# benjaminrwilson/range-view-3d-detection

Hardware: AMD Instinct MI355X
Metric: sweeps/sec (fwd+bwd, 64x2048x5 range image) (higher is better)
Workload: dtype bf16

## Files before the change

include/rv3d.h:

```cpp
#ifndef RV3D_H_
#define RV3D_H_

#include <stdint.h>

#ifdef __cplusplus
extern "C" {
#endif

typedef void* rvStream;

int rv_version(void);
const char* rv_last_error(void);

typedef struct {
    int32_t kh, kw;
    int32_t stride_w;
    int32_t pad_h, pad_w;
    int32_t cu, cv;
} rvTapGeom;

int32_t rv_pad_channels(int32_t c);

int64_t rv_packed_weight_bytes(const rvTapGeom* g);

int rv_pack_weight(const rvTapGeom* g, const float* T, void* gather_w, void* scatter_w, rvStream stream);

int64_t rv_pack_batch_entry_bytes(void);
int rv_pack_batch_fill(const rvTapGeom* g, const float* T, void* gather_w, void* scatter_w, void* host_entries);
int rv_pack_batch(const void* dev_table, int32_t n_entries, rvStream stream);

int rv_fold_geom(const rvTapGeom* g, rvTapGeom* folded);
int rv_pack_weight_folded(const rvTapGeom* g, const float* T, void* gather_w_folded, rvStream stream);
int rv_pack_batch_fill_folded(const rvTapGeom* g, const float* T, void* gather_w_folded, void* host_entry);
int rv_unfold_weight_grad(const rvTapGeom* g, const float* dT_folded, float* dT, int32_t accumulate, rvStream stream);

int rv_unpack_weight_grad(const rvTapGeom* g, const float* packed, float* dT, int32_t accumulate, rvStream stream);

#define RV_IN_AFFINE 1
#define RV_IN_RELU 2
#define RV_OUT_F32 4
#define RV_OUT_BIAS 8
#define RV_OUT_STATS 16
#define RV_OUT_ACCUM 32
#define RV_OUT_RELU 64
#define RV_OUT_RES_RELU 256
#define RV_WGRAD_TORCH_LAYOUT 128
#define RV_SEL_SMALL_GRIDS (1 << 20)
#define RV_SEL_SMALL_GRIDS6 (1 << 21)
#define RV_SEL_NO_GEN6 (1 << 22)
#define RV_SEL_NO_GEN5 (1 << 23)
#define RV_SEL_NO_POINTWISE (1 << 24)
#define RV_SEL_NO_POINTWISE_BWD (1 << 25)
#define RV_SEL_MASK (63 << 20)

typedef struct {
    int32_t N, H, Wu, Wv;
    int32_t ld_src, ld_dst;
    int32_t flags;
} rvTapShape;

int32_t rv_tap_stats_rows(const rvTapGeom* g, const rvTapShape* s, int32_t scatter);
int rv_tap_launch_info(const rvTapGeom* g, const rvTapShape* s, int32_t scatter, int32_t* host_info);
#define RV_STATS_SCRATCH_ROWS 128

int rv_tap_gather(const rvTapGeom* g, const rvTapShape* s, const void* V, const float* in_scale,
                  const float* in_shift, const void* gather_w, const float* bias, void* U,
                  float* stats_partial, rvStream stream);

int rv_tap_scatter(const rvTapGeom* g, const rvTapShape* s, const void* U, const float* in_scale,
                   const float* in_shift, const void* scatter_w, const float* bias, void* V,
                   float* stats_partial, rvStream stream);

int rv_tap_residual(const rvTapGeom* g, const rvTapShape* s, int32_t scatter, const void* src, const void* w, const float* bias,
                    const void* res, int32_t ld_res, void* dst, rvStream stream);

typedef struct rvBnbEpilogue {
    const void* y;
    int32_t ld_y;
    int32_t flags;
    const float* scale;
    const float* shift;
    const float* mean;
    const float* invstd;
    float* partial;
} rvBnbEpilogue;
int32_t rv_tap_bnb_rows(const rvTapGeom* g, const rvTapShape* s, int32_t scatter);
int rv_tap_data_grad_bnb(const rvTapGeom* g, const rvTapShape* s, int32_t scatter, const void* dout, const void* w, void* dx,
                         const rvBnbEpilogue* e, rvStream stream);

int64_t rv_tap_wgrad_workspace_bytes(const rvTapGeom* g, const rvTapShape* s);
int rv_tap_wgrad_info(const rvTapGeom* g, const rvTapShape* s, int32_t* host_info);
int rv_tap_wgrad(const rvTapGeom* g, const rvTapShape* s, const void* U, int32_t ld_u, const void* V, int32_t ld_v,
                 const float* in_scale, const float* in_shift, int32_t v_affine, float* dT_packed,
                 void* workspace, rvStream stream);

int rv_reduce_rows(const float* partial, int32_t rows, int32_t cols, float* out, rvStream stream);
int rv_reduce_rows_count(const float* partial, int32_t rows, int32_t cols, float count, float* out, float* out_copy, rvStream stream);
int rv_bn_finalize(const float* partial, int32_t rows, int32_t c, int64_t count, const float* gamma,
                   const float* beta, float eps, float momentum, float* running_mean, float* running_var,
                   float* scale, float* shift, float* mean, float* invstd, rvStream stream);
int rv_bn_fold_eval(int32_t c, const float* gamma, const float* beta, const float* running_mean,
                    const float* running_var, float eps, float* scale, float* shift, rvStream stream);

#define RV_EW_RELU_A 1
#define RV_EW_RELU_B 2
#define RV_EW_RELU_OUT 4
// ... 354 lines not shown
```

range_view_3d_detection_amd/_lib.py:

```python

from __future__ import annotations

import ctypes
import os
import re
import functools
from typing import Dict, List, Optional, Tuple

import torch

_HERE = os.path.dirname(os.path.abspath(__file__))
LIB_PATH = os.environ.get("RV3D_LIB") or os.path.join(_HERE, "librv3d_hip.so")
LIB_PATH_F16 = os.environ.get("RV3D_LIB_F16") or os.path.join(_HERE, "librv3d_hip_f16.so")
HEADER_PATH = os.path.join(os.path.dirname(_HERE), "include", "rv3d.h")
COMPANION_HEADERS = ("rv3d_render.h",)
OPTIM_HEADERS = ("rv3d_optim.h",)
AVERAGE_ENTRIES = ("rv_adamw_step_groups_avg", "rv_average_tensors")

IN_AFFINE, IN_RELU, OUT_F32, OUT_BIAS, OUT_STATS, OUT_ACCUM, OUT_RELU = 1, 2, 4, 8, 16, 32, 64
OUT_RES_RELU = 256
WGRAD_TORCH_LAYOUT = 128
SEL_SMALL_GRIDS, SEL_SMALL_GRIDS6, SEL_NO_GEN6, SEL_NO_GEN5, SEL_NO_POINTWISE, SEL_NO_POINTWISE_BWD = 1 << 20, 1 << 21, 1 << 22, 1 << 23, 1 << 24, 1 << 25
SELECT = 0
EW_RELU_A, EW_RELU_B, EW_RELU_OUT = 1, 2, 4
BNB_RELU_Z, BNB_RES_ACCUM, BNB_Y_FROM_INPUT = 1, 2, 4
ADAM_AMSGRAD, ADAM_MAXIMIZE = 1, 2
WNMS_MERGE_SUPPRESSED, WNMS_SCORE_KEEPER, WNMS_NMS_GE, WNMS_MERGE_GE = 1, 2, 4, 8
EW_PASS_COMBINE, EW_PASS_MASK_GRAD, EW_PASS_BN_FINALIZE, EW_PASS_BWD_REDUCE, EW_PASS_BWD_REDUCE_PAIR, EW_PASS_BWD_FINALIZE, EW_PASS_BWD_APPLY, EW_PASS_BWD_APPLY_PAIR = range(8)
EW_FORM_COMB, EW_FORM_ROWS, EW_FORM_OCTET, EW_FORM_LEAN, EW_FORM_FUSED_FINALIZE, EW_FORM_TWO_STAGE = range(1, 7)
STATS_SCRATCH_ROWS = 128


class TapGeom(ctypes.Structure):
    _fields_ = [(n, ctypes.c_int32) for n in ("kh", "kw", "stride_w", "pad_h", "pad_w", "cu", "cv")]


class TapShape(ctypes.Structure):
    _fields_ = [(n, ctypes.c_int32) for n in ("N", "H", "Wu", "Wv", "ld_src", "ld_dst", "flags")]

    def __init__(self, *args, **kw) -> None:
        super().__init__(*args, **kw)
        self.flags |= SELECT


class select:

    def __init__(self, flags: int) -> None:
        self.flags = flags

    def __enter__(self):
        global SELECT
        self.old, SELECT = SELECT, SELECT | self.flags
        return self

    def __exit__(self, *exc):
        global SELECT
        SELECT = self.old


class BnbEpilogue(ctypes.Structure):

    _fields_ = [("y", ctypes.c_void_p), ("ld_y", ctypes.c_int32), ("flags", ctypes.c_int32), ("scale", ctypes.c_void_p), ("shift", ctypes.c_void_p),
                ("mean", ctypes.c_void_p), ("invstd", ctypes.c_void_p), ("partial", ctypes.c_void_p)]


class TargetLevel(ctypes.Structure):

    _fields_ = [("stride", ctypes.c_int32), ("use_range", ctypes.c_int32), ("lower", ctypes.c_double), ("upper", ctypes.c_double)]


class TargetOut(ctypes.Structure):

    _fields_ = [(n, ctypes.c_void_p) for n in ("labels", "panoptics", "reg_targets", "points_per_obj")]


# ... 271 lines not shown
```

range_view_3d_detection_amd/csrc/tapconv.h:

```cpp
#pragma once
#include "common.h"

constexpr int kMaxTaps = 24;
constexpr int kMaxPhases = 4;
constexpr int RV_OUT_BNB = 1 << 16;

struct TapTable {
    int32_t ntaps[kMaxPhases];
    int32_t w_first[kMaxPhases];
    int32_t dw_min[kMaxPhases], dw_max[kMaxPhases];
    int32_t w_tile[kMaxPhases];
    int32_t dh_min, rows;
    int8_t dh[kMaxPhases][kMaxTaps];
    int8_t dw[kMaxPhases][kMaxTaps];
    int8_t ky[kMaxPhases][kMaxTaps];
    int8_t kx[kMaxPhases][kMaxTaps];
};

struct TapConvArgs {
    const bf16_t* src;
    void* dst;
    const bf16_t* w;
    const float* in_scale;
    const float* in_shift;
    const float* bias;
    float* stats;
    int32_t N, H, W_src, W_dst;
    int32_t C_src, C_dst;
    int32_t ld_src, ld_dst;
    int32_t phases, step;
    int32_t m_tiles;
    int32_t h_tiles;
    int32_t total_tiles, n_tiles, tiles_per_xcd;
    int32_t lds_a_elems;
    int32_t lds_tab_offset;
    int32_t flags;
    int32_t sel;
    const bf16_t* bnb_y;
    const float *bnb_scale, *bnb_shift, *bnb_mean, *bnb_invstd;
    float* bnb_partial;
    int32_t ld_bnb_y, bnb_flags;
    const bf16_t* res;
    int32_t ld_res;
    int32_t stats_per_wg;
    TapTable tt;
};

int rv_build_tap_table(const rvTapGeom* g, bool scatter, TapTable* tt, int* phases, int* step);

struct TapPlan {
    int gen;
    int bn, ks;
    int mt, nt;
    int epi;
    int pair, slices;
    int grid_x, grid_y;
    size_t lds;
    int stats_rows;
    int bnb_rows;
    int32_t info[4];
    bool scatter;
    TapConvArgs args;
};

bool rv_tapconv2_plan(TapPlan* p);
int rv_tapconv2_launch(const TapPlan& p, hipStream_t stream);
bool rv_tapconv4_plan(TapPlan* p);
int rv_tapconv4_launch(const TapPlan& p, hipStream_t stream);
bool rv_tapconv5_plan(TapPlan* p);
int rv_tapconv5_launch(const TapPlan& p, hipStream_t stream);
bool rv_tapconv6_plan(TapPlan* p);
int rv_tapconv6_launch(const TapPlan& p, hipStream_t stream);
bool rv_pointwise_plan(TapPlan* p);
int rv_pointwise_launch(const TapPlan& p, hipStream_t stream);
```

range_view_3d_detection_amd/csrc/tapconv6.hip:

```cpp
#include <stdlib.h>

#include "common.h"
#include "tapconv.h"

namespace {

constexpr int kTC = 32;
constexpr int kTR = 16;
constexpr int kBK = 32;
constexpr int kBN = 128;
constexpr int kPitch = 36;
constexpr int kHaloRows = 18;
constexpr int kHaloInstr = (kHaloRows * kPitch + 15) / 16;
constexpr int kHaloBytes = kHaloInstr * 1024;
constexpr int kPiece = kBN * kBK * 2;
constexpr int kNRing = 8;
#ifndef RV_T6_AHEAD
#define RV_T6_AHEAD 4
#endif
constexpr int kAhead = RV_T6_AHEAD;
constexpr int kRing = 2 * kHaloBytes;
constexpr int kScratch = kRing + kNRing * kPiece;
constexpr int kTab = kScratch + 1024;
constexpr int kStatAcc = kTab + 32 * 4;
constexpr int kBnbAcc = kStatAcc + 8 * 4 * 16 * 2 * 4;
constexpr int kLds = kBnbAcc + 256 * 4;
constexpr int kMinTaps = kAhead + 2 > 6 ? kAhead + 2 : 6;

__device__ __attribute__((aligned(256))) uint32_t g_zero_page6[64];

typedef __attribute__((address_space(3))) void lds_void_t;
typedef const __attribute__((address_space(1))) void glb_void_t;

constexpr int wait_count(int U) {
    if (U > kAhead) return kAhead - 1;
    int n = 0;
    for (int u = U - kAhead + 1; u <= U; ++u) n += (u >= 0 && u < 3) ? 2 : 0;
    return kAhead - 1 + n;
}

template <int EPI>
__global__ __launch_bounds__(512, 2) void tapconv6_kernel(const TapConvArgs a) {
    extern __shared__ __attribute__((aligned(16))) uint8_t smem[];
    const int tid = threadIdx.x, lane = tid & 63;
    const int wave = __builtin_amdgcn_readfirstlane(tid >> 6);
    const int wr = wave >> 1, wc = wave & 1;
    const int l15 = lane & 15, lg = lane >> 4;
    constexpr int kHaloPer = 6;
    constexpr int kHaloPerTile = kHaloPer / 3;

    const int gy = a.n_tiles;
    const int xcd = blockIdx.x & 7, wslot = blockIdx.x >> 3, nslots = gridDim.x >> 3;
    auto stat_slot = [&]() { return (float*)(smem + kStatAcc) + (wave * 4 * 16 + l15) * 2; };
    if (a.stats_per_wg && lg == 0) {
        float* stat_acc = stat_slot();
#pragma unroll
        for (int j = 0; j < 4; ++j) {
            stat_acc[j * 32] = 0.f;
            stat_acc[j * 32 + 1] = 0.f;
        }
    }
    if ((EPI == 1) && a.stats_per_wg && tid < 256)
        ((float*)(smem + kBnbAcc))[tid] = 0.f;
    for (int k = 0;; ++k) {
    const int xslot = wslot + nslots * k;
    if (xslot >= a.tiles_per_xcd * gy) break;
    const int tile = xcd * a.tiles_per_xcd + xslot / gy;
    if (tile >= a.total_tiles) continue;
    const int n0 = (xslot % gy) * kBN;
    int bx = tile;
    const int tc = bx % a.m_tiles;
    bx /= a.m_tiles;
    const int th = bx % a.h_tiles;
    bx /= a.h_tiles;
    const int n = bx % a.N;
    const int ph = bx / a.N;
    const int m0 = tc * kTC, h0 = th * kTR;
    const int T = a.tt.ntaps[ph];
    const int nkc = a.C_src / kBK;
    const int nkt = T * nkc;
    const int HW = kTC + a.tt.dw_max[ph] - a.tt.dw_min[ph];
    const int HR = kTR + a.tt.rows - 1;

    const bf16_t* src_img = a.src + ((int64_t)n * a.H * a.W_src) * a.ld_src;
    int* tap_tab = (int*)(smem + kTab);
    if (tid < 16) tap_tab[tid] = tid < T ? (a.tt.dh[ph][tid] - a.tt.dh_min) * kPitch + (a.tt.dw[ph][tid] - a.tt.dw_min[ph]) : 0;
    __syncthreads();
    const int ncol = T / a.tt.rows;
    const int sh0 = __builtin_amdgcn_readfirstlane(tap_tab[0]);
    const int sh_dcol = ncol > 1 ? __builtin_amdgcn_readfirstlane(tap_tab[1]) - sh0 : 0;
    const int sh_drow = ncol < T ? __builtin_amdgcn_readfirstlane(tap_tab[ncol]) - __builtin_amdgcn_readfirstlane(tap_tab[ncol - 1]) : 0;
    const int row_base = h0 + a.tt.dh_min, col_base = m0 + a.tt.dw_min[ph];

    const int s_row = lane >> 2, s_slot = lane & 3;
    const int kq8 = (s_slot ^ (((s_row >> 2) & 1) << 1)) * 8;
    const bf16_t* zero = (const bf16_t*)g_zero_page6 + s_slot * 8;
    const int64_t w_img = (int64_t)a.C_dst * a.C_src;
    const bf16_t* w_ph = a.w + (int64_t)a.tt.w_first[ph] * w_img;
    const int b_voff = (n0 + wave * 16 + s_row) * a.C_src + kq8;
    int bq = 0, bt = 0;
    int b_so = 0;
    auto stage_b = [&](int j) {
        const int so = __builtin_amdgcn_readfirstlane(b_so);
        const bf16_t* p = w_ph + so + b_voff;
        __builtin_amdgcn_global_load_lds((glb_void_t*)p, (lds_void_t*)(smem + kRing + (j & (kNRing - 1)) * kPiece + wave * 1024), 16, 0, 0);
        const bool go = bq + 1 < nkt;
        const bool wrap = bt + 1 == T;
        bq += go ? 1 : 0;
        b_so += go ? (wrap ? kBK - (T - 1) * (int)w_img : (int)w_img) : 0;
        bt = go ? (wrap ? 0 : bt + 1) : bt;
    };
    int hoff[kHaloPer];
#pragma unroll
    for (int i = 0; i < kHaloPer; ++i) {
        const int q = wave + 8 * i;
        const int p = q * 16 + s_row;
        const int hr = (p * 1821) >> 16, hc = p - hr * kPitch;
        const int row = row_base + hr, col = col_base + hc;
        const int bad = (q >= kHaloInstr) | (hc >= HW) | (hr >= HR) | (row < 0) | (row >= a.H) | (col < 0) | (col >= a.W_src);
        hoff[i] = ((row * a.W_src + col) * a.ld_src + kq8) | -bad;
    }
    auto stage_halo = [&](int buf, int i, int kc) {
        const int q = wave + 8 * i;
        const bf16_t* src = hoff[i] >= 0 ? src_img + (hoff[i] + kc * kBK) : zero;
        const int dst = q < kHaloInstr ? buf * kHaloBytes + q * 1024 : kScratch;
        __builtin_amdgcn_global_load_lds((glb_void_t*)src, (lds_void_t*)(smem + dst), 16, 0, 0);
    };

    const int p_lane = (4 * wr) * kPitch + l15;
    const int b_rd = (wc * 64 + l15) * 64 + ((lg ^ (((l15 >> 2) & 1) << 1)) * 16);
    bf16x8 fa[4], fb[4];
    int a_b0 = 0, a_b1 = 0;
    auto addr_a = [&](int halo_byte, int shift) {
        const int p = p_lane + shift;
        a_b0 = halo_byte + p * 64 + ((lg ^ (((p >> 2) & 1) << 1)) * 16);
        a_b1 = a_b0 ^ 32;
    };
    auto read_a = [&](int mq) {
#pragma unroll
        for (int rr = 0; rr < 2; ++rr)
#pragma unroll
            for (int cc = 0; cc < 2; ++cc)
                fa[rr * 2 + cc] = *(const bf16x8*)(smem + (((2 * mq + rr) & 1) ? a_b1 : a_b0) + (2 * mq + rr) * (kPitch * 64) + cc * 1024);
    };
    auto read_b = [&](int j) {
#pragma unroll
        for (int jj = 0; jj < 4; ++jj) fb[jj] = *(const bf16x8*)(smem + kRing + (j & (kNRing - 1)) * kPiece + jj * 1024 + b_rd);
    };

    f32x4 acc[8][4];
#pragma unroll
    for (int i = 0; i < 8; ++i)
#pragma unroll
        for (int j = 0; j < 4; ++j) acc[i][j] = f32x4{0.f, 0.f, 0.f, 0.f};

#define RV_PHASE_COMPUTE(MQ)                                                                            \
    __builtin_amdgcn_s_barrier();                                                                       \
    asm volatile("s_waitcnt lgkmcnt(0)" ::: "memory");                                                  \
    __builtin_amdgcn_sched_barrier(0);                                                                  \
    __builtin_amdgcn_s_setprio(1);                                                                      \
    _Pragma("unroll") for (int i = 0; i < 4; ++i) _Pragma("unroll") for (int jj = 0; jj < 4; ++jj)      \
        acc[(MQ) * 4 + i][jj] = RV_MFMA_16x16x32(fa[i], fb[jj], acc[(MQ) * 4 + i][jj], 0, 0, 0);        \
    __builtin_amdgcn_s_setprio(0);                                                                      \
    __builtin_amdgcn_sched_barrier(0);                                                                  \
    __builtin_amdgcn_s_barrier();

#pragma unroll
    for (int i = 0; i < kHaloPer; ++i) stage_halo(0, i, 0);
#pragma unroll
    for (int j = 0; j < kAhead; ++j) stage_b(j);
    asm volatile("s_waitcnt vmcnt(0)" ::: "memory");
    __builtin_amdgcn_s_barrier();
    if (wave >= 4) __builtin_amdgcn_s_barrier();

    int kt = 0, kc = 0;
    int sh = sh0, ix = 0;
#define RV_KTILE(U, HALO)                                                                                         \
    {                                                                                                              \
        constexpr int W = (HALO) ? wait_count(U) : kAhead - 1;                                                     \
        const int hbuf = (kc + 1) & 1;                                                                             \
        stage_b(kt + kAhead);                                                                                      \
        if constexpr ((HALO) && (U) <= 2) stage_halo(hbuf, kHaloPerTile * (U), kc + 1);                            \
        addr_a((kc & 1) * kHaloBytes, sh);                                                                         \
        read_b(kt);                                                                                                \
        __builtin_amdgcn_sched_barrier(0);                                                                         \
        read_a(0);                                                                                                 \
        RV_PHASE_COMPUTE(0);                                                                                       \
        read_a(1);                                                                                                 \
        if constexpr ((HALO) && (U) <= 2) stage_halo(hbuf, kHaloPerTile * (U) + 1, kc + 1);                        \
        asm volatile("s_waitcnt vmcnt(%0)" ::"n"(W) : "memory");                                                   \
        RV_PHASE_COMPUTE(1);                                                                                       \
        ++kt;                                                                                                      \
        const bool wrap = ix + 1 == ncol;                                                                          \
        sh += wrap ? sh_drow : sh_dcol;                                                                            \
        ix = wrap ? 0 : ix + 1;                                                                                    \
    }
    for (; kc + 1 < nkc; ++kc) {
        RV_KTILE(0, true)
        RV_KTILE(1, true)
        RV_KTILE(2, true)
        RV_KTILE(3, true)
        RV_KTILE(4, true)
        RV_KTILE(5, true)
        if (T > 6) RV_KTILE(6, true)
        if (T > 7) RV_KTILE(7, true)
        if (T > 8) RV_KTILE(8, true)
        for (int t = 9; t < T; ++t) RV_KTILE(9, true)
        sh = sh0;
        ix = 0;
    }
    for (int t = 0; t < T; ++t) RV_KTILE(9, false)
#undef RV_KTILE
#undef RV_PHASE_COMPUTE
    if (wave < 4) __builtin_amdgcn_s_barrier();
    asm volatile("s_waitcnt vmcnt(0)" ::: "memory");
    __syncthreads();

    const int Wm = a.W_dst / a.phases;
#pragma unroll
    for (int i = 0; i < 8; ++i) {
        const bool row_ok = h0 + 4 * wr + (i >> 1) < a.H;
#pragma unroll
        for (int r = 0; r < 4; ++r) {
            const int m = m0 + (i & 1) * 16 + lg * 4 + r;
            if (m >= Wm || !row_ok) {
#pragma unroll
                for (int j = 0; j < 4; ++j) acc[i][j][r] = 0.f;
            }
        }
    }
    if (a.flags & RV_OUT_STATS) {
        float* prow = a.stats + ((int64_t)(tile * 4 + wr) * 2) * a.C_dst;
        float* stat_acc = stat_slot();
#pragma unroll
        for (int j = 0; j < 4; ++j) {
            float s = 0.f, q = 0.f;
#pragma unroll
            for (int i = 0; i < 8; ++i)
#pragma unroll
                for (int r = 0; r < 4; ++r) {
                    const float v = acc[i][j][r];
                    s += v;
                    q += v * v;
                }
            s += __shfl_xor(s, 16, 64);
            q += __shfl_xor(q, 16, 64);
            s += __shfl_xor(s, 32, 64);
            q += __shfl_xor(q, 32, 64);
            const int c = n0 + wc * 64 + j * 16 + l15;
            if (lg == 0) {
                if (a.stats_per_wg) {
                    stat_acc[j * 32] += s;
                    stat_acc[j * 32 + 1] += q;
                } else {
                    prow[c] = s;
                    prow[a.C_dst + c] = q;
                }
            }
        }
    }
    if (a.flags & RV_OUT_BIAS) {
        const bool relu_out = (a.flags & RV_OUT_RELU) != 0;
#pragma unroll
        for (int j = 0; j < 4; ++j) {
            const float b = a.bias[n0 + wc * 64 + j * 16 + l15];
#pragma unroll
            for (int i = 0; i < 8; ++i)
#pragma unroll
                for (int r = 0; r < 4; ++r) acc[i][j][r] = relu_out ? fmaxf(acc[i][j][r] + b, 0.f) : acc[i][j][r] + b;
        }
    }
    constexpr int kEpi = kBN + 8;
    bf16_t* epi = (bf16_t*)smem;
#pragma unroll
    for (int i = 0; i < 8; ++i)
#pragma unroll
        for (int j = 0; j < 4; ++j)
#pragma unroll
            for (int r = 0; r < 4; ++r) {
                const int pm = (4 * wr + (i >> 1)) * kTC + (i & 1) * 16 + lg * 4 + r;
                const int pc = wc * 64 + j * 16 + l15;
                epi[pm * kEpi + pc] = f2bf(acc[i][j][r]);
            }
    constexpr int kChunks = kBN / 8;
    constexpr bool accum = EPI == 2;
    constexpr bool bnb = EPI == 1;
    static_assert(EPI >= 0 && EPI <= 2, "the masked last-writer epilogue (three prefetches per pass) stays on tapconv5");
    constexpr int kStoreThreads = 512;
    constexpr int kPasses = kTR * kTC * kChunks / kStoreThreads;
    int st = tid;
    asm volatile("" : "+v"(st));
    float bsc[8], bsh[8], bmu[8], bis[8], s0[8], s1[8];
    if (bnb) {
        const int c = n0 + (st & (kChunks - 1)) * 8;
#pragma unroll
        for (int j = 0; j < 8; ++j) {
            bsc[j] = a.bnb_scale[c + j];
            bsh[j] = a.bnb_shift[c + j];
            bmu[j] = a.bnb_mean[c + j];
            bis[j] = a.bnb_invstd[c + j];
            s0[j] = 0.f;
            s1[j] = 0.f;
        }
    }
    constexpr int kRound = 8, kRounds = kPasses / kRound;
    constexpr bool pre = bnb || accum;
    u32x4 yv[pre ? 2 : 1][pre ? kRound : 1];
    auto prefetch = [&](int r, int buf) {
#pragma unroll
        for (int i = 0; i < kRound; ++i) {
            const int q = st + (r * kRound + i) * kStoreThreads, pm = q / kChunks, c8 = q - pm * kChunks;
            const int rr = pm / kTC, mm = pm - rr * kTC;
            const int m = min(m0 + mm, Wm - 1), hh = min(h0 + rr, a.H - 1), c = n0 + c8 * 8;
            const int64_t px = ((int64_t)(n * a.H + hh) * a.W_dst) + (a.phases * m + ph);
            yv[pre ? buf : 0][pre ? i : 0] = bnb ? *(const u32x4*)(a.bnb_y + px * a.ld_bnb_y + c) : *(const u32x4*)(a.res + px * a.ld_res + c);
        }
    };
    if (pre) prefetch(0, 0);
    __syncthreads();
#pragma unroll
    for (int r = 0; r < kRounds; ++r) {
        if (pre && r + 1 < kRounds) prefetch(r + 1, (r + 1) & 1);
#pragma unroll
        for (int i = 0; i < kRound; ++i) {
            const int q = st + (r * kRound + i) * kStoreThreads;
            const int pm = q / kChunks, c8 = q - pm * kChunks;
            const int rr = pm / kTC, mm = pm - rr * kTC;
            const int m = m0 + mm, c = n0 + c8 * 8, hh = h0 + rr;
            if (m >= Wm || hh >= a.H) continue;
            u32x4 v = *(const u32x4*)(epi + pm * kEpi + c8 * 8);
            const int64_t px = ((int64_t)(n * a.H + hh) * a.W_dst) + (a.phases * m + ph);
            bf16_t* p = (bf16_t*)a.dst + px * a.ld_dst + c;
            const u32x4 pv = yv[pre ? (r & 1) : 0][pre ? i : 0];
            if (accum) {
#pragma unroll
                for (int j = 0; j < 4; ++j) v[j] = pack_bf2(bf_lo(v[j]) + bf_lo(pv[j]), bf_hi(v[j]) + bf_hi(pv[j]));
                if (a.flags & RV_OUT_RES_RELU) {
#pragma unroll
                    for (int j = 0; j < 4; ++j) v[j] = pack_bf2(fmaxf(bf_lo(v[j]), 0.f), fmaxf(bf_hi(v[j]), 0.f));
                }
            }
// ... 2 lines not shown
#pragma unroll
                for (int j = 0; j < 4; ++j) {
                    const float y0 = bf_lo(pv[j]), y1 = bf_hi(pv[j]);
                    float g0 = bf_lo(v[j]), g1 = bf_hi(v[j]);
                    if (a.bnb_flags & 1) {
                        g0 = y0 * bsc[2 * j] + bsh[2 * j] > 0.f ? g0 : 0.f;
                        g1 = y1 * bsc[2 * j + 1] + bsh[2 * j + 1] > 0.f ? g1 : 0.f;
                    }
                    s0[2 * j] += g0;
                    s0[2 * j + 1] += g1;
                    s1[2 * j] += g0 * ((y0 - bmu[2 * j]) * bis[2 * j]);
                    s1[2 * j + 1] += g1 * ((y1 - bmu[2 * j + 1]) * bis[2 * j + 1]);
                }
            }
        }
    }
    if (bnb) {
        __syncthreads();
        float* red = (float*)smem;
        constexpr int kSW = kStoreThreads / 64;
#pragma unroll
        for (int j = 0; j < 8; ++j) {
#pragma unroll
            for (int d = kChunks; d < 64; d <<= 1) {
                s0[j] += __shfl_xor(s0[j], d, 64);
                s1[j] += __shfl_xor(s1[j], d, 64);
            }
        }
        if (lane < kChunks) {
#pragma unroll
            for (int j = 0; j < 8; ++j) {
                red[((st >> 6) * kChunks + lane) * 16 + j] = s0[j];
                red[((st >> 6) * kChunks + lane) * 16 + 8 + j] = s1[j];
            }
        }
        __syncthreads();
        const int chunk = st >> 4, jj = st & 15;
        if (chunk < kChunks) {
            float sum = 0.f;
#pragma unroll
            for (int w = 0; w < kSW; ++w) sum += red[(w * kChunks + chunk) * 16 + jj];
            if (a.stats_per_wg) ((float*)(smem + kBnbAcc))[st] += sum;
            else a.bnb_partial[((int64_t)tile * 2 + (jj >> 3)) * a.C_dst + n0 + chunk * 8 + (jj & 7)] = sum;
        }
    }
    __syncthreads();
    }
    if ((EPI == 1) && a.stats_per_wg && tid < 256) {
        const int so = tid, chunk = so >> 4, jj = so & 15;
        a.bnb_partial[((int64_t)(xcd * (nslots / gy) + wslot / gy) * 2 + (jj >> 3)) * a.C_dst + (wslot % gy) * kBN + chunk * 8 + (jj & 7)] =
            ((const float*)(smem + kBnbAcc))[so];
    }
    if ((a.flags & RV_OUT_STATS) && a.stats_per_wg && lg == 0) {
        float* prow = a.stats + ((int64_t)((xcd * (nslots / gy) + wslot / gy) * 4 + wr) * 2) * a.C_dst;
        const float* stat_acc = stat_slot();
        const int c0 = (wslot % gy) * kBN + wc * 64 + l15;
#pragma unroll
        for (int j = 0; j < 4; ++j) {
            prow[c0 + j * 16] = stat_acc[j * 32];
            prow[a.C_dst + c0 + j * 16] = stat_acc[j * 32 + 1];
        }
    }
}


}


bool rv_tapconv6_plan(TapPlan* p) {
    TapConvArgs* a = &p->args;
    if (a->step != 1) return false;
    if (a->flags & (RV_IN_AFFINE | RV_IN_RELU | RV_OUT_F32)) return false;
    if ((a->flags & RV_OUT_BNB) && (a->flags & RV_OUT_ACCUM)) return false;
    if (a->C_src % kBK != 0 || a->C_dst % kBN != 0) return false;
    const int wm_total = a->W_dst / a->phases;
    if (wm_total < kTC || a->H < kTR) return false;
    if (kTR + a->tt.rows - 1 > kHaloRows) return false;
    for (int r = 0; r < a->phases; ++r) {
        if (a->tt.ntaps[r] < kMinTaps || a->tt.ntaps[r] > 16) return false;
        const int hw = kTC + a->tt.dw_max[r] - a->tt.dw_min[r];
        if (hw > 34) return false;
        const int T = a->tt.ntaps[r], nrow = a->tt.rows;
        if (T % nrow != 0) return false;
        const int ncol = T / nrow;
        auto shift = [&](int t) { return (a->tt.dh[r][t] - a->tt.dh_min) * kPitch + (a->tt.dw[r][t] - a->tt.dw_min[r]); };
        const int dcol = ncol > 1 ? shift(1) - shift(0) : 0, drow = ncol < T ? shift(ncol) - shift(ncol - 1) : 0;
        int sh = shift(0), ix = 0;
        for (int t = 1; t < T; ++t) {
            if (ix + 1 == ncol) {
                sh += drow;
                ix = 0;
            } else {
                sh += dcol;
                ++ix;
            }
            if (sh != shift(t)) return false;
        }
    }
    if ((int64_t)a->H * a->W_src * a->ld_src >= (1ll << 31) || (int64_t)kMaxTaps * a->C_dst * a->C_src >= (1ll << 31)) return false;
    a->m_tiles = rv_ceil_div(wm_total, kTC);
    a->h_tiles = rv_ceil_div(a->H, kTR);
    a->total_tiles = a->m_tiles * a->h_tiles * a->N * a->phases;
    a->n_tiles = a->C_dst / kBN;
    a->tiles_per_xcd = rv_ceil_div(a->total_tiles, 8);
    if ((int64_t)a->total_tiles * a->n_tiles < ((a->sel & RV_SEL_SMALL_GRIDS6) ? 1 : rv_cu_count())) return false;
    int grid = 8 * a->tiles_per_xcd * a->n_tiles;
    if (grid > rv_cu_count()) grid = rv_persistent_grid();
    const int nslots = grid / 8;
    a->stats_per_wg = (nslots % a->n_tiles == 0) ? 1 : 0;
    p->gen = 6;
    p->epi = (a->flags & RV_OUT_BNB) ? 1 : ((a->flags & RV_OUT_ACCUM) ? 2 : 0);
    p->grid_x = grid;
    p->stats_rows = a->stats_per_wg ? (grid / a->n_tiles) * 4 : a->total_tiles * 4;
    p->bnb_rows = a->stats_per_wg ? grid / a->n_tiles : a->total_tiles;
    p->lds = (size_t)kLds;
    const size_t epi = (size_t)kTR * kTC * (kBN + 8) * sizeof(bf16_t);
    if (p->lds < epi) p->lds = epi;
    p->info[0] = 6, p->info[1] = kBN, p->info[2] = a->total_tiles, p->info[3] = a->n_tiles;
    return true;
}

template <int EPI>
static int launch6(const TapPlan& p, hipStream_t stream) {
    RV_LDS_OPT_IN(160 * 1024, tapconv6_kernel<EPI>);
    hipLaunchKernelGGL((tapconv6_kernel<EPI>), dim3(p.grid_x), dim3(512), p.lds, stream, p.args);
    RV_CHECK_LAUNCH("tapconv6_kernel");
    return 0;
}

int rv_tapconv6_launch(const TapPlan& p, hipStream_t stream) {
    return p.epi == 0 ? launch6<0>(p, stream) : p.epi == 1 ? launch6<1>(p, stream) : launch6<2>(p, stream);
}
```

range_view_3d_detection_amd/engine.py:

```python

from __future__ import annotations

import ctypes
import os
import weakref
from dataclasses import dataclass, field
from typing import Dict, List, Optional, Sequence, Tuple, Union

import torch
from torch import Tensor, nn

from . import _lib as L
from .images import Image, ImageCache

BN_EPS = 1e-5
BN_MOMENTUM = 0.1

SYNC_BN: Optional[bool] = None
SYNC_WORLD1 = os.environ.get("RV3D_SYNC_WORLD1") is not None


def _dist_world() -> int:
    if torch.distributed.is_available() and torch.distributed.is_initialized():
        return torch.distributed.get_world_size()
# ... 367 lines not shown
                   L.ptr(self.bn.shift), None, 0, None, None, out.ptr(), out.ld, L.EW_RELU_A if self.relu else 0,
                   L.stream_ptr())
            self.plain = out
        return self.plain


Operand = Union[Act, Lazy]


def ptr_ld(a: Optional[Act]) -> tuple:
    return (a.ptr(), a.ld) if a is not None else (None, 0)


def partial_rows(rows: int, cp: int, device) -> Tensor:
    return torch.empty((rows + L.STATS_SCRATCH_ROWS, 2, cp), dtype=torch.float32, device=device)


@dataclass(eq=False, slots=True)
class BnbSums:
    partial: Tensor
    rows: int
    over: Act
    masked: bool = False


@dataclass(eq=False, slots=True)
class PendingGrad:
    dout: Act
    mask: Optional[Act] = None
    res: Optional[Tuple[Act, bool]] = None
    owned: bool = False
    sums: Optional[BnbSums] = None


@dataclass(eq=False, slots=True)
class PendingMeta:
    dgeo: Act
    feat: Act
    partial: Tensor
    rows: int


@dataclass(eq=False, slots=True)
class PendingHeadFinal:
    head: tuple
    partial: Tensor
    rows: int
    dY: Act
    wp: Tensor


MATERIALIZE_FOR_DMA = True
BNB_FUSE = True


def _dma_generation(geom, n: int, h: int, wu: int, wv: int, ld_src: int, ld_dst: int, scatter: bool) -> int:
    info = L.tap_launch_info(geom, L.TapShape(n, h, wu, wv, ld_src, ld_dst, 0), scatter)
    return info[0] if info is not None else 0


def _dma_eligible(geom, n: int, h: int, wu: int, wv: int, ld_src: int, ld_dst: int, scatter: bool) -> bool:
    return _dma_generation(geom, n, h, wu, wv, ld_src, ld_dst, scatter) in (4, 5, 6)


MATERIALIZE_FOR_POINTWISE = True
MATERIALIZE_POINTWISE_C = (256,)


def _materialize_operand(x, layer, src, wu: int, wv: int, out, out_f32: bool, eval_bn) -> bool:
    if not (isinstance(x, Lazy) and MATERIALIZE_FOR_DMA and not out_f32):
        return False
    g, form = layer.geom, layer.fwd_form
    if g.kh * g.kw > 1 and _dma_eligible(g, src.N, src.H, wu, wv, src.ld, pad32(layer.c_out), form == "scatter"):
        return True
    if (MATERIALIZE_FOR_POINTWISE and g.kh * g.kw == 1 and layer.bias is None and eval_bn is None and pad32(layer.c_in) in MATERIALIZE_POINTWISE_C
            and _dma_generation(g, src.N, src.H, wu, wv, pad32(layer.c_in), out.ld if out is not None else pad32(layer.c_out), form == "scatter") == 7):
        return True
    return (form == "gather" and g.stride_w > 1 and g.kh * g.kw > 1 and layer.fold_geom() is not None and src.ld == src.cp
            and src.W == g.stride_w * wu and _dma_eligible(layer.fold_geom(), src.N, src.H, wu, wu, g.stride_w * src.ld, pad32(layer.c_out), False))


_LAYERS: "weakref.WeakSet[TapLayer]" = weakref.WeakSet()
_PACK_TABLES: Dict[tuple, Tensor] = {}
BATCH_PACK = True
FOLD_STRIDED = True
FORMS = ("gather", "scatter")


def image_slot(form: Optional[str], kind: Optional[str] = None) -> tuple:
    return (kind or ("folded" if form == "folded" else "weight"), form, L.operand_tag())


def prepack_stale() -> None:
    def is_stale(l: "TapLayer") -> bool:
        held = [e.current for e in l.images.entries() if e.slot[0] == "weight"]
        w = l.weight
        return bool(held) and not any(held) and l.in_perm is None and w.requires_grad and w.is_cuda and w.dtype == torch.float32 and w.is_contiguous()

    stale = sorted(filter(is_stale, _LAYERS), key=id) if BATCH_PACK else []
    if len(stale) < 2:
        return
    with L.operand("bf16"):
        imgs = {l: {f: l.image_buffer(f) for f in (*FORMS, "folded") if f != "folded" or l.images.held(image_slot(f))} for l in stale}
        folded = [l for l in stale if "folded" in imgs[l]]
        key = tuple((id(l), l.weight.data_ptr(), *(img.data_ptr() for img in imgs[l].values())) for l in stale)
        n_entries = 2 * len(stale) + len(folded)
# ... 234 lines not shown


class Op:
    def backward(self, t: Tape) -> None:
        raise NotImplementedError


def _operand_parts(x: Operand) -> Tuple[Act, Optional[Tensor], Optional[Tensor], int]:
    if isinstance(x, Lazy):
        return x.raw, x.bn.scale, x.bn.shift, L.IN_AFFINE | (L.IN_RELU if x.relu else 0)
    return x, None, None, 0


class ConvOp(Op):

    def __init__(self, t: Tape, layer: TapLayer, x: Operand, stats: bool = False, out_f32: bool = False,
                 out: Optional[Act] = None, need_input_grad: bool = True, precomputed: Optional[Tuple[Optional[Tensor], int]] = None,
                 eval_bn: Optional[nn.Module] = None, relu_out: bool = False, residual: Optional[Act] = None,
                 res_relu: bool = False) -> None:
        self.layer, self.x, self.need_input_grad = layer, x, need_input_grad
        self.eval_bn = eval_bn
        assert residual is None or (eval_bn is not None and not out_f32 and not stats)
        self.pos_first: Optional["SmallKOp"] = None
        src, sc, sh, flags = _operand_parts(x)
        form = layer.fwd_form
        g = layer.geom
        wu, wv = (src.W // g.stride_w, src.W) if form == "gather" else (src.W, src.W * g.stride_w)
        w_out = wu if form == "gather" else wv
        assert src.cp == pad32(layer.c_in), (src.cp, layer.c_in)
        self.x_plain = None
        if _materialize_operand(x, layer, src, wu, wv, out, out_f32, eval_bn):
            self.x_plain = src = x.materialized()
            sc = sh = None
            flags = 0
        self.out_f32 = out_f32
        if out_f32:
            self.out_t = torch.empty((src.N, src.H, w_out, pad32(layer.c_out)), dtype=torch.float32, device=t.device)
            dst_ptr, ld_dst = L.ptr(self.out_t), self.out_t.stride(2)
            flags |= L.OUT_F32
            self.out = None
        else:
            self.out = out if out is not None else Act.empty(src.N, src.H, w_out, layer.c_out, t.device)
            dst_ptr, ld_dst = self.out.ptr(), self.out.ld
        bias = layer.bias
        if eval_bn is not None:
            assert bias is None and not stats and not t.training
            flags |= L.OUT_BIAS | (L.OUT_RELU if relu_out else 0) | (L.OUT_RES_RELU if residual is not None and res_relu else 0)
            bias_p = None
        elif bias is not None:
            flags |= L.OUT_BIAS
            bias_p = layer.padded_bias()
        else:
            bias_p = None
        self.shape = L.TapShape(src.N, src.H, wu, wv, src.ld, ld_dst, flags | (L.OUT_STATS if stats else 0))
        lg, lshape, wp = g, self.shape, None
        gf = layer.fold_geom() if (form == "gather" and g.stride_w > 1 and sc is None and flags & (L.IN_AFFINE | L.IN_RELU) == 0) else None
        if gf is not None and src.ld == src.cp and src.W == g.stride_w * wu and _dma_eligible(gf, src.N, src.H, wu, wu, g.stride_w * src.ld, ld_dst, False):
            lg = gf
            lshape = L.TapShape(src.N, src.H, wu, wu, g.stride_w * src.ld, ld_dst, self.shape.flags)
            wp = layer.packed_folded() if eval_bn is None else "folded"
        self.partial = None
        self.rows = 0
        if stats:
            self.rows = L.load().rv_tap_stats_rows(lg, lshape, 1 if form == "scatter" else 0)
            if self.rows < 0:
                raise L.RvError("rv_tap_stats_rows: " + L.load().rv_last_error().decode())
            self.partial = partial_rows(self.rows, pad32(layer.c_out), t.device)
        if eval_bn is not None:
            wp, bias_p = layer.packed_eval("folded" if isinstance(wp, str) else form, eval_bn)
        elif wp is None:
            wp = layer.packed(form)
        call = lambda: L.call("rv_tap_" + form, lg, lshape, src.ptr(), L.ptr(sc), L.ptr(sh),
                              L.ptr(wp), L.ptr(bias_p), dst_ptr, L.ptr(self.partial), L.stream_ptr())
        if residual is not None:
            assert sc is None and flags & (L.IN_AFFINE | L.IN_RELU) == 0 and residual.cp == self.out.cp and residual.pixels == self.out.pixels
            call = lambda: L.call("rv_tap_residual", lg, lshape, 1 if form == "scatter" else 0, src.ptr(),
                                  L.ptr(wp), L.ptr(bias_p), residual.ptr(), residual.ld, dst_ptr, L.stream_ptr())
        if precomputed is not None:
            assert out is not None and not out_f32 and bias is None
            self.partial, self.rows = precomputed
        elif PROFILE is not None:
            _launch(tap_kernel_name(lg, lshape, form == "scatter"), tap_flops(g, self.shape), call, tap_bytes(g, self.shape))
        else:
            call()
        self.count = src.N * src.H * w_out
        t.ops.append(self)

    def backward(self, t: Tape) -> None:
        from . import engine_bwd

        if self.eval_bn is not None:
            raise L.RvError("this conv ran with an eval-mode BatchNorm folded into its weights (inference): there is no backward")
        engine_bwd.conv_backward(self, t)


class BnOp(Op):

    def __init__(self, t: Tape, conv: ConvOp, bn: nn.BatchNorm2d, relu: bool = True, reduced: Optional[Tensor] = None) -> None:
        self.conv = conv
        self.sync_world = 1
        c = bn.num_features
        cp = pad32(c)
        dev = t.device
        gamma, beta = _padded(bn.weight, cp), _padded(bn.bias, cp)
        scale = torch.empty(cp, dtype=torch.float32, device=dev)
        shift = torch.empty(cp, dtype=torch.float32, device=dev)
        self.gamma_p = gamma
# ... 338 lines not shown
```

range_view_3d_detection_amd/engine_bwd.py:

```python

from __future__ import annotations

import ctypes
import os
from dataclasses import dataclass
from typing import Optional, Sequence, Tuple

import torch
from torch import Tensor

from . import _lib as L
from . import engine as E
from .engine import Act, Lazy, Tape, pad32


def grad_act_like(o: Act, g: Tensor) -> Act:
    nhwc = g.permute(0, 2, 3, 1)
    if g.dtype == torch.bfloat16 and g.shape[1] == o.cp and nhwc.is_contiguous():
        return Act(nhwc, o.c)
    out = Act.empty(o.N, o.H, o.W, o.c, g.device, zero=(g.shape[1] != o.cp))
    out.data[..., : g.shape[1]].copy_(nhwc)
    return out


def seed_f32_output_grad(t: Tape, op: "E.ConvOp", g: Tensor) -> None:
    c = op.layer.c_out
    n, h, w = op.out_t.shape[:3]
    act = Act.empty(n, h, w, c, g.device, zero=(c % 32 != 0))
    act.data[..., :c].copy_(g.permute(0, 2, 3, 1))
    t.raw_grad[id(op)] = act
    if op.layer.bias is not None:
        if c < 8:
            t.add_param_grad(op.layer.bias, g.float().permute(0, 2, 3, 1).sum(dim=2).sum(dim=(0, 1)))
        else:
            t.add_param_grad(op.layer.bias, g.float().sum(dim=(0, 2, 3)))


def _conv_out_grad(op: "E.ConvOp", t: Tape) -> Optional[Act]:
    if op.out_f32:
        return t.raw_grad.get(id(op))
    g = t.raw_grad.get(id(op.out))
    if g is None and id(op.out) in t.grads and id(op.out) in t.written:
        g = t.grads[id(op.out)]
    return g


def conv_backward(op: "E.ConvOp", t: Tape) -> None:
    dout = _conv_out_grad(op, t)
    if dout is None:
        return
    _release_held_wgrads(t)
    layer, g = op.layer, op.layer.geom
    src, sc, sh, in_flags = E._operand_parts(op.x)
    if op.x_plain is not None:
        src, sc, sh, in_flags = op.x_plain, None, None, 0
    fwd = layer.fwd_form
    bwd = "scatter" if fwd == "gather" else "gather"
    sp = op.shape
    fused_first = POS_BWD_FUSE and op.pos_first is not None and op.need_input_grad and t.training
    early_ready = None
    if fused_first:
        _wait_chained_wgrad(t)
        _pos_pair_backward(op, t, dout)
    elif op.need_input_grad and _head_final_eligible(op, t, dout):
        _head_final_sums(op, t, dout)
        return
    elif op.need_input_grad:
        if isinstance(op.x, Lazy):
            dst, accumulate = t.lazy_grad_target(op.x)
        else:
            dst, accumulate = t.grad_buffer(op.x)
        shape = L.TapShape(sp.N, sp.H, sp.Wu, sp.Wv, dout.ld, dst.ld, L.OUT_ACCUM if accumulate else 0)
        bg, bshape = g, shape
        gf = layer.fold_geom() if (bwd == "gather" and g.stride_w > 1) else None
        if (gf is not None and dout.ld == dout.cp and dout.W == g.stride_w * sp.Wu
                and E._dma_eligible(gf, sp.N, sp.H, sp.Wu, sp.Wu, g.stride_w * dout.ld, dst.ld, False)):
            bg = gf
            bshape = L.TapShape(sp.N, sp.H, sp.Wu, sp.Wu, g.stride_w * dout.ld, dst.ld, shape.flags)
            wp = layer.packed_folded()
        elif (E.FOLD_STRIDED and bwd == "scatter" and g.stride_w == 2 and g.kh == 1 and g.kw == 1 and g.pad_w == 0 and dst.ld == dst.cp
              and dst.W == 2 * sp.Wu):
            if not accumulate:
                dst.data.zero_()
            bg = L.TapGeom(1, 1, 1, 0, 0, g.cu, g.cv)
            bshape = L.TapShape(sp.N, sp.H, sp.Wu, sp.Wu, dout.ld, 2 * dst.ld, shape.flags)
            wp = layer.packed(bwd)
        else:
            wp = layer.packed(bwd)
        call = lambda: L.call("rv_tap_" + bwd, bg, bshape, dout.ptr(), None, None, L.ptr(wp), None,
                              dst.ptr(), None, L.stream_ptr())
        if E.BNB_FUSE and bg is g and isinstance(op.x, Lazy) and not accumulate and op.x.bn.mean is not None:
            rows = L.load().rv_tap_bnb_rows(g, shape, 1 if bwd == "scatter" else 0)
            if rows > 0:
                lz, st = op.x, op.x.bn
                partial = E.partial_rows(rows, dst.cp, t.device)
                epi = L.BnbEpilogue(lz.raw.ptr(), lz.raw.ld, L.BNB_RELU_Z if lz.relu else 0, L.ptr(st.scale), L.ptr(st.shift),
                                    L.ptr(st.mean), L.ptr(st.invstd), L.ptr(partial))
                call = lambda: L.call("rv_tap_data_grad_bnb", g, shape, 1 if bwd == "scatter" else 0, dout.ptr(),
                                      L.ptr(wp), dst.ptr(), epi, L.stream_ptr())
                t.pending[id(lz)].sums = E.BnbSums(partial, rows, dst)
        if E.OVERLAP_WGRAD and E.EARLY_WGRAD_FILL > 0:
            info = L.tap_launch_info(bg, bshape, bwd == "scatter")
            if info is not None and info[0] == 6:
                wg_tiles, cus = info[2] * info[3], E.cu_count(t.device)
                if wg_tiles / (cus * ((wg_tiles + cus - 1) // cus)) < E.EARLY_WGRAD_FILL:
                    early_ready = torch.cuda.Event()
                    early_ready.record()
                    t.chained_wgrad = None
        _wait_chained_wgrad(t)
        if E.PROFILE is not None:
            E._launch(E.tap_kernel_name(bg, bshape, bwd == "scatter"), E.tap_flops(g, shape), call, E.tap_bytes(g, shape))
        else:
            call()
        if not isinstance(op.x, Lazy):
            t.mark_written(op.x)
    u, v, v_affine = (dout, src, 1) if fwd == "gather" else (src, dout, 0)
    wshape = L.TapShape(sp.N, sp.H, sp.Wu, sp.Wv, 0, 0, in_flags | L.WGRAD_TORCH_LAYOUT)
    wg, wsh, ld_v = g, wshape, v.ld
    gfw = layer.fold_geom() if (g.stride_w > 1 and sc is None and in_flags == 0 and v.ld == v.cp and v.W == g.stride_w * sp.Wu) else None
    if gfw is not None:
        wg, wsh, ld_v = gfw, L.TapShape(sp.N, sp.H, sp.Wu, sp.Wu, 0, 0, L.WGRAD_TORCH_LAYOUT), g.stride_w * v.ld

    def run_wgrad() -> None:
        ws_bytes = L.load().rv_tap_wgrad_workspace_bytes(wg, wsh)
        ws = torch.empty(ws_bytes, dtype=torch.uint8, device=t.device)
# ... 348 lines not shown
```

Baseline: 43.23.

## Add half-height four-wave tapconv6 variant selected for measured-winning conv shapes

Templates the gen6 tap-convolution kernel on a HALF mode that uses 8-row tiles, 4 waves, a smaller B ring and prefetch depth, and a compact LDS layout. This allows more workgroups per CU and doubles the grid for better load balance on mid-sized layers. A hard-coded table of layer shapes (channels, taps, epilogue, pixel count) picks when the half form is used by default via a new selector flag passed from the forward and backward engines. The cost is less reuse per tile and more halo overhead per output row. The shape table is tuned to this network's layer sizes.

```diff
diff --git a/include/rv3d.h b/include/rv3d.h
--- a/include/rv3d.h
+++ b/include/rv3d.h
@@ -51,7 +51,10 @@
 #define RV_SEL_NO_GEN5 (1 << 23)
 #define RV_SEL_NO_POINTWISE (1 << 24)
 #define RV_SEL_NO_POINTWISE_BWD (1 << 25)
-#define RV_SEL_MASK (63 << 20)
+#define RV_SEL_NO_HALF6 (1 << 26)
+#define RV_SEL_HALF6 (1 << 27)
+#define RV_SEL_HALF6_MEASURED (1 << 28)
+#define RV_SEL_MASK (511 << 20)
 
 typedef struct {
     int32_t N, H, Wu, Wv;
diff --git a/range_view_3d_detection_amd/_lib.py b/range_view_3d_detection_amd/_lib.py
--- a/range_view_3d_detection_amd/_lib.py
+++ b/range_view_3d_detection_amd/_lib.py
@@ -21,6 +21,7 @@
 OUT_RES_RELU = 256
 WGRAD_TORCH_LAYOUT = 128
 SEL_SMALL_GRIDS, SEL_SMALL_GRIDS6, SEL_NO_GEN6, SEL_NO_GEN5, SEL_NO_POINTWISE, SEL_NO_POINTWISE_BWD = 1 << 20, 1 << 21, 1 << 22, 1 << 23, 1 << 24, 1 << 25
+SEL_NO_HALF6, SEL_HALF6, SEL_HALF6_MEASURED = 1 << 26, 1 << 27, 1 << 28
 SELECT = 0
 EW_RELU_A, EW_RELU_B, EW_RELU_OUT = 1, 2, 4
 BNB_RELU_Z, BNB_RES_ACCUM, BNB_Y_FROM_INPUT = 1, 2, 4
diff --git a/range_view_3d_detection_amd/csrc/tapconv.h b/range_view_3d_detection_amd/csrc/tapconv.h
--- a/range_view_3d_detection_amd/csrc/tapconv.h
+++ b/range_view_3d_detection_amd/csrc/tapconv.h
@@ -53,6 +53,7 @@
     int bn, ks;
     int mt, nt;
     int epi;
+    int half;
     int pair, slices;
     int grid_x, grid_y;
     size_t lds;
diff --git a/range_view_3d_detection_amd/csrc/tapconv6.hip b/range_view_3d_detection_amd/csrc/tapconv6.hip
--- a/range_view_3d_detection_amd/csrc/tapconv6.hip
+++ b/range_view_3d_detection_amd/csrc/tapconv6.hip
@@ -6,41 +6,55 @@
 namespace {
 
 constexpr int kTC = 32;
-constexpr int kTR = 16;
 constexpr int kBK = 32;
 constexpr int kBN = 128;
 constexpr int kPitch = 36;
-constexpr int kHaloRows = 18;
-constexpr int kHaloInstr = (kHaloRows * kPitch + 15) / 16;
-constexpr int kHaloBytes = kHaloInstr * 1024;
 constexpr int kPiece = kBN * kBK * 2;
-constexpr int kNRing = 8;
 #ifndef RV_T6_AHEAD
 #define RV_T6_AHEAD 4
 #endif
-constexpr int kAhead = RV_T6_AHEAD;
-constexpr int kRing = 2 * kHaloBytes;
-constexpr int kScratch = kRing + kNRing * kPiece;
-constexpr int kTab = kScratch + 1024;
-constexpr int kStatAcc = kTab + 32 * 4;
-constexpr int kBnbAcc = kStatAcc + 8 * 4 * 16 * 2 * 4;
-constexpr int kLds = kBnbAcc + 256 * 4;
-constexpr int kMinTaps = kAhead + 2 > 6 ? kAhead + 2 : 6;
+
+template <bool HALF>
+struct Tile6 {
+    static constexpr int kTR = HALF ? 8 : 16;
+    static constexpr int kWaves = HALF ? 4 : 8;
+    static constexpr int kThreads = 64 * kWaves;
+    static constexpr int kWR = kWaves / 2;
+    static constexpr int kWInstr = 8 / kWaves;
+    static constexpr int kHaloRows = kTR + 2;
+    static constexpr int kHaloInstr = (kHaloRows * kPitch + 15) / 16;
+    static constexpr int kHaloBytes = kHaloInstr * 1024;
+    static constexpr int kNRing = HALF ? 4 : 8;
+    static constexpr int kAhead = HALF ? 3 : RV_T6_AHEAD;
+    static constexpr int kRing = 2 * kHaloBytes;
+    static constexpr int kScratch = kRing + kNRing * kPiece;
+    static constexpr int kTab = HALF ? kRing + (kNRing - 1) * kPiece : kScratch + 1024;
+    static constexpr int kStatAcc = HALF ? kScratch : kTab + 32 * 4;
+    static constexpr int kBnbAcc = HALF ? kStatAcc : kStatAcc + kWaves * 4 * 16 * 2 * 4;
+    static constexpr int kLds = HALF ? kStatAcc + kWaves * 4 * 16 * 2 * 4 : kBnbAcc + 256 * 4;
+    static constexpr int kMinTaps = kAhead + 2 > 6 ? kAhead + 2 : 6;
+    static constexpr int kEpiBytes = kTR * kTC * (kBN + 8) * 2;
+    static_assert(kAhead < kNRing && kLds >= kEpiBytes && kLds >= kBnbAcc + 256 * 4, "LDS layout");
+    static_assert(!HALF || (kLds <= 80 * 1024 && kEpiBytes <= kTab), "half form: two workgroups per CU; the tap table outlives no staged tile");
+
+    static constexpr int wait_count(int U) {
+        if (U > kAhead) return kWInstr * (kAhead - 1);
+        int n = 0;
+        for (int u = U - kAhead + 1; u <= U; ++u) n += (u >= 0 && u < 3) ? 2 : 0;
+        return kWInstr * (kAhead - 1) + n;
+    }
+};
 
 __device__ __attribute__((aligned(256))) uint32_t g_zero_page6[64];
 
 typedef __attribute__((address_space(3))) void lds_void_t;
 typedef const __attribute__((address_space(1))) void glb_void_t;
 
-constexpr int wait_count(int U) {
-    if (U > kAhead) return kAhead - 1;
-    int n = 0;
-    for (int u = U - kAhead + 1; u <= U; ++u) n += (u >= 0 && u < 3) ? 2 : 0;
-    return kAhead - 1 + n;
-}
-
-template <int EPI>
-__global__ __launch_bounds__(512, 2) void tapconv6_kernel(const TapConvArgs a) {
+template <int EPI, bool HALF>
+__global__ __launch_bounds__(Tile6<HALF>::kThreads, 2) void tapconv6_kernel(const TapConvArgs a) {
+    using G = Tile6<HALF>;
+    constexpr int kTR = G::kTR, kWaves = G::kWaves, kWR = G::kWR, kWInstr = G::kWInstr, kHaloInstr = G::kHaloInstr, kHaloBytes = G::kHaloBytes;
+    constexpr int kNRing = G::kNRing, kAhead = G::kAhead, kRing = G::kRing, kScratch = G::kScratch, kTab = G::kTab, kStatAcc = G::kStatAcc, kBnbAcc = G::kBnbAcc;
     extern __shared__ __attribute__((aligned(16))) uint8_t smem[];
     const int tid = threadIdx.x, lane = tid & 63;
     const int wave = __builtin_amdgcn_readfirstlane(tid >> 6);
@@ -103,17 +117,21 @@
     auto stage_b = [&](int j) {
         const int so = __builtin_amdgcn_readfirstlane(b_so);
         const bf16_t* p = w_ph + so + b_voff;
-        __builtin_amdgcn_global_load_lds((glb_void_t*)p, (lds_void_t*)(smem + kRing + (j & (kNRing - 1)) * kPiece + wave * 1024), 16, 0, 0);
+#pragma unroll
+        for (int h = 0; h < kWInstr; ++h)
+            __builtin_amdgcn_global_load_lds((glb_void_t*)(p + h * (kWaves * 16) * a.C_src),
+                                             (lds_void_t*)(smem + kRing + (j & (kNRing - 1)) * kPiece + (wave + h * kWaves) * 1024), 16, 0, 0);
         const bool go = bq + 1 < nkt;
         const bool wrap = bt + 1 == T;
         bq += go ? 1 : 0;
         b_so += go ? (wrap ? kBK - (T - 1) * (int)w_img : (int)w_img) : 0;
         bt = go ? (wrap ? 0 : bt + 1) : bt;
     };
+    auto halo_q = [&](int i) { return HALF ? min(wave + kWaves * i, kHaloInstr - 1) : wave + kWaves * i; };
     int hoff[kHaloPer];
 #pragma unroll
     for (int i = 0; i < kHaloPer; ++i) {
-        const int q = wave + 8 * i;
+        const int q = halo_q(i);
         const int p = q * 16 + s_row;
         const int hr = (p * 1821) >> 16, hc = p - hr * kPitch;
         const int row = row_base + hr, col = col_base + hc;
@@ -121,9 +139,9 @@
         hoff[i] = ((row * a.W_src + col) * a.ld_src + kq8) | -bad;
     }
     auto stage_halo = [&](int buf, int i, int kc) {
-        const int q = wave + 8 * i;
+        const int q = halo_q(i);
         const bf16_t* src = hoff[i] >= 0 ? src_img + (hoff[i] + kc * kBK) : zero;
-        const int dst = q < kHaloInstr ? buf * kHaloBytes + q * 1024 : kScratch;
+        const int dst = (HALF || q < kHaloInstr) ? buf * kHaloBytes + q * 1024 : kScratch;
         __builtin_amdgcn_global_load_lds((glb_void_t*)src, (lds_void_t*)(smem + dst), 16, 0, 0);
     };
 
@@ -171,13 +189,13 @@
     for (int j = 0; j < kAhead; ++j) stage_b(j);
     asm volatile("s_waitcnt vmcnt(0)" ::: "memory");
     __builtin_amdgcn_s_barrier();
-    if (wave >= 4) __builtin_amdgcn_s_barrier();
+    if (!HALF && wave >= 4) __builtin_amdgcn_s_barrier();
 
     int kt = 0, kc = 0;
     int sh = sh0, ix = 0;
 #define RV_KTILE(U, HALO)                                                                                         \
     {                                                                                                              \
-        constexpr int W = (HALO) ? wait_count(U) : kAhead - 1;                                                     \
+        constexpr int W = (HALO) ? G::wait_count(U) : kWInstr * (kAhead - 1);                                                    \
         const int hbuf = (kc + 1) & 1;                                                                             \
         stage_b(kt + kAhead);                                                                                      \
         if constexpr ((HALO) && (U) <= 2) stage_halo(hbuf, kHaloPerTile * (U), kc + 1);                            \
@@ -212,7 +230,7 @@
     for (int t = 0; t < T; ++t) RV_KTILE(9, false)
 #undef RV_KTILE
 #undef RV_PHASE_COMPUTE
-    if (wave < 4) __builtin_amdgcn_s_barrier();
+    if (!HALF && wave < 4) __builtin_amdgcn_s_barrier();
     asm volatile("s_waitcnt vmcnt(0)" ::: "memory");
     __syncthreads();
 
@@ -230,7 +248,7 @@
         }
     }
     if (a.flags & RV_OUT_STATS) {
-        float* prow = a.stats + ((int64_t)(tile * 4 + wr) * 2) * a.C_dst;
+        float* prow = a.stats + ((int64_t)(tile * kWR + wr) * 2) * a.C_dst;
         float* stat_acc = stat_slot();
 #pragma unroll
         for (int j = 0; j < 4; ++j) {
@@ -286,7 +304,7 @@
     constexpr bool accum = EPI == 2;
     constexpr bool bnb = EPI == 1;
     static_assert(EPI >= 0 && EPI <= 2, "the masked last-writer epilogue (three prefetches per pass) stays on tapconv5");
-    constexpr int kStoreThreads = 512;
+    constexpr int kStoreThreads = G::kThreads;
     constexpr int kPasses = kTR * kTC * kChunks / kStoreThreads;
     int st = tid;
     asm volatile("" : "+v"(st));
@@ -395,7 +413,7 @@
             ((const float*)(smem + kBnbAcc))[so];
     }
     if ((a.flags & RV_OUT_STATS) && a.stats_per_wg && lg == 0) {
-        float* prow = a.stats + ((int64_t)((xcd * (nslots / gy) + wslot / gy) * 4 + wr) * 2) * a.C_dst;
+        float* prow = a.stats + ((int64_t)((xcd * (nslots / gy) + wslot / gy) * kWR + wr) * 2) * a.C_dst;
         const float* stat_acc = stat_slot();
         const int c0 = (wslot % gy) * kBN + wc * 64 + l15;
 #pragma unroll
@@ -410,7 +428,28 @@
 }
 
 
-bool rv_tapconv6_plan(TapPlan* p) {
+struct HalfWin {
+    int c_src, c_dst, taps, epi;
+    int64_t pixels;
+};
+constexpr int64_t kPx = 4 * 64;
+constexpr HalfWin kHalfWins[] = {
+    {128, 128, 9, 0, kPx * 2656}, {128, 128, 9, 1, kPx * 2656}, {128, 128, 9, 2, kPx * 2656},
+    {128, 128, 9, 0, kPx * 664},  {128, 128, 9, 1, kPx * 664},  {128, 128, 9, 2, kPx * 664},
+    {512, 128, 9, 2, kPx * 664},  {256, 128, 9, 0, kPx * 664},  {256, 128, 6, 0, kPx * 664},
+    {128, 128, 6, 0, kPx * 2656}, {128, 128, 6, 0, kPx * 664},
+};
+
+static bool half_form_wins(const TapConvArgs& a, int epi) {
+    for (const HalfWin& w : kHalfWins)
+        if (w.c_src == a.C_src && w.c_dst == a.C_dst && w.taps == a.tt.ntaps[0] && w.epi == epi && w.pixels == (int64_t)a.N * a.H * a.W_dst) return true;
+    return false;
+}
+
+template <bool HALF>
+static bool plan6(TapPlan* p) {
+    using G = Tile6<HALF>;
+    constexpr int kTR = G::kTR;
     TapConvArgs* a = &p->args;
     if (a->step != 1) return false;
     if (a->flags & (RV_IN_AFFINE | RV_IN_RELU | RV_OUT_F32)) return false;
@@ -418,9 +457,9 @@
     if (a->C_src % kBK != 0 || a->C_dst % kBN != 0) return false;
     const int wm_total = a->W_dst / a->phases;
     if (wm_total < kTC || a->H < kTR) return false;
-    if (kTR + a->tt.rows - 1 > kHaloRows) return false;
+    if (kTR + a->tt.rows - 1 > G::kHaloRows) return false;
     for (int r = 0; r < a->phases; ++r) {
-        if (a->tt.ntaps[r] < kMinTaps || a->tt.ntaps[r] > 16) return false;
+        if (a->tt.ntaps[r] < G::kMinTaps || a->tt.ntaps[r] > 16) return false;
         const int hw = kTC + a->tt.dw_max[r] - a->tt.dw_min[r];
         if (hw > 34) return false;
         const int T = a->tt.ntaps[r], nrow = a->tt.rows;
@@ -446,31 +485,40 @@
     a->total_tiles = a->m_tiles * a->h_tiles * a->N * a->phases;
     a->n_tiles = a->C_dst / kBN;
     a->tiles_per_xcd = rv_ceil_div(a->total_tiles, 8);
-    if ((int64_t)a->total_tiles * a->n_tiles < ((a->sel & RV_SEL_SMALL_GRIDS6) ? 1 : rv_cu_count())) return false;
+    constexpr int kPerCu = HALF ? 2 : 1;
+    if ((int64_t)a->total_tiles * a->n_tiles < ((a->sel & RV_SEL_SMALL_GRIDS6) ? 1 : kPerCu * rv_cu_count())) return false;
     int grid = 8 * a->tiles_per_xcd * a->n_tiles;
-    if (grid > rv_cu_count()) grid = rv_persistent_grid();
+    if (grid > kPerCu * rv_cu_count()) grid = kPerCu * rv_persistent_grid();
     const int nslots = grid / 8;
     a->stats_per_wg = (nslots % a->n_tiles == 0) ? 1 : 0;
     p->gen = 6;
     p->epi = (a->flags & RV_OUT_BNB) ? 1 : ((a->flags & RV_OUT_ACCUM) ? 2 : 0);
+    p->half = HALF ? 1 : 0;
     p->grid_x = grid;
-    p->stats_rows = a->stats_per_wg ? (grid / a->n_tiles) * 4 : a->total_tiles * 4;
+    p->stats_rows = a->stats_per_wg ? (grid / a->n_tiles) * G::kWR : a->total_tiles * G::kWR;
     p->bnb_rows = a->stats_per_wg ? grid / a->n_tiles : a->total_tiles;
-    p->lds = (size_t)kLds;
-    const size_t epi = (size_t)kTR * kTC * (kBN + 8) * sizeof(bf16_t);
-    if (p->lds < epi) p->lds = epi;
+    p->lds = (size_t)G::kLds;
     p->info[0] = 6, p->info[1] = kBN, p->info[2] = a->total_tiles, p->info[3] = a->n_tiles;
     return true;
 }
 
-template <int EPI>
+bool rv_tapconv6_plan(TapPlan* p) {
+    const TapPlan shape = *p;
+    const int sel = shape.args.sel;
+    if (!(sel & RV_SEL_NO_HALF6) && (sel & (RV_SEL_HALF6 | RV_SEL_HALF6_MEASURED)) && plan6<true>(p) && ((sel & RV_SEL_HALF6) || half_form_wins(p->args, p->epi))) return true;
+    *p = shape;
+    return plan6<false>(p);
+}
+
+template <int EPI, bool HALF>
 static int launch6(const TapPlan& p, hipStream_t stream) {
-    RV_LDS_OPT_IN(160 * 1024, tapconv6_kernel<EPI>);
-    hipLaunchKernelGGL((tapconv6_kernel<EPI>), dim3(p.grid_x), dim3(512), p.lds, stream, p.args);
+    RV_LDS_OPT_IN(160 * 1024, tapconv6_kernel<EPI, HALF>);
+    hipLaunchKernelGGL((tapconv6_kernel<EPI, HALF>), dim3(p.grid_x), dim3(Tile6<HALF>::kThreads), p.lds, stream, p.args);
     RV_CHECK_LAUNCH("tapconv6_kernel");
     return 0;
 }
 
 int rv_tapconv6_launch(const TapPlan& p, hipStream_t stream) {
-    return p.epi == 0 ? launch6<0>(p, stream) : p.epi == 1 ? launch6<1>(p, stream) : launch6<2>(p, stream);
-}
+    if (!p.half) return p.epi == 0 ? launch6<0, false>(p, stream) : p.epi == 1 ? launch6<1, false>(p, stream) : launch6<2, false>(p, stream);
+    return p.epi == 0 ? launch6<0, true>(p, stream) : p.epi == 1 ? launch6<1, true>(p, stream) : launch6<2, true>(p, stream);
+}
diff --git a/range_view_3d_detection_amd/engine.py b/range_view_3d_detection_amd/engine.py
--- a/range_view_3d_detection_amd/engine.py
+++ b/range_view_3d_detection_amd/engine.py
@@ -443,6 +443,7 @@
 
 MATERIALIZE_FOR_DMA = True
 BNB_FUSE = True
+TAP_SELECT = L.SEL_HALF6_MEASURED
 
 
 def _dma_generation(geom, n: int, h: int, wu: int, wv: int, ld_src: int, ld_dst: int, scatter: bool) -> int:
@@ -783,7 +784,7 @@
             bias_p = layer.padded_bias()
         else:
             bias_p = None
-        self.shape = L.TapShape(src.N, src.H, wu, wv, src.ld, ld_dst, flags | (L.OUT_STATS if stats else 0))
+        self.shape = L.TapShape(src.N, src.H, wu, wv, src.ld, ld_dst, flags | (L.OUT_STATS if stats else 0) | TAP_SELECT)
         lg, lshape, wp = g, self.shape, None
         gf = layer.fold_geom() if (form == "gather" and g.stride_w > 1 and sc is None and flags & (L.IN_AFFINE | L.IN_RELU) == 0) else None
         if gf is not None and src.ld == src.cp and src.W == g.stride_w * wu and _dma_eligible(gf, src.N, src.H, wu, wu, g.stride_w * src.ld, ld_dst, False):
diff --git a/range_view_3d_detection_amd/engine_bwd.py b/range_view_3d_detection_amd/engine_bwd.py
--- a/range_view_3d_detection_amd/engine_bwd.py
+++ b/range_view_3d_detection_amd/engine_bwd.py
@@ -70,7 +70,7 @@
             dst, accumulate = t.lazy_grad_target(op.x)
         else:
             dst, accumulate = t.grad_buffer(op.x)
-        shape = L.TapShape(sp.N, sp.H, sp.Wu, sp.Wv, dout.ld, dst.ld, L.OUT_ACCUM if accumulate else 0)
+        shape = L.TapShape(sp.N, sp.H, sp.Wu, sp.Wv, dout.ld, dst.ld, (L.OUT_ACCUM if accumulate else 0) | E.TAP_SELECT)
         bg, bshape = g, shape
         gf = layer.fold_geom() if (bwd == "gather" and g.stride_w > 1) else None
         if (gf is not None and dout.ld == dout.cp and dout.W == g.stride_w * sp.Wu
```

Result: no change. 43.21 (-0.0%).
